# ska-sa/dc_sand

Hardware: AMD Instinct MI355X
Metric: Gcoeff/s (complex weights) 64ant x 1024beam x 32768chan per GPU (higher is better)
Workload: dtype f32

## Files before the change

### dc_sand_amd/csrc/bf_capi.hip

```cpp

#include "../../include/dcs_beamformer.h"
#ifdef DCS_PROBES
#include "../../include/dcs_probes.h"
#endif

#include <hip/hip_runtime.h>

#include <cmath>
#include <cstdio>
#include <cstdlib>
#include <cstring>
#include <new>

#include "../../include/dcs_stream_staging.h"
#include "bf_kernels.h"
#include "bf_ctx_ext.h"
#include "bf_stream_ext.h"

static_assert(sizeof(dcs_delay_vals) == 16, "delay_vals must be 4 x fp32 (BeamformerParameters.h:61-66)");

#define DCS_TRY(expr)                          \
    do {                                       \
        hipError_t _e = (expr);                \
        if (_e != hipSuccess) return (int)_e;  \
// ... 43 lines not shown
    k.dHalfChannels = p->nr_channels / 2.0;
    k.dDenominator = (double)D;
    return k;
}

int verify_div3(dcs_bf_consts *k)
{
    uint32_t *d_cnt = nullptr;
    uint32_t h_cnt = 1;
    hipError_t e = hipMalloc((void **)&d_cnt, sizeof(uint32_t));
    if (e != hipSuccess) return (int)e;
    e = hipMemset(d_cnt, 0, sizeof(uint32_t));
    if (e == hipSuccess) e = bf_launch_verify_div3(k->fDenominator, k->fRcpDenominator, d_cnt, nullptr);
    if (e == hipSuccess) e = hipMemcpy(&h_cnt, d_cnt, sizeof(uint32_t), hipMemcpyDeviceToHost);
    (void)hipFree(d_cnt);
    if (e != hipSuccess) return (int)e;
    k->uDiv3Exact = (h_cnt == 0u) ? 1u : 0u;
    return DCS_OK;
}

}

constexpr int kSideStreams = 4;
struct dcs_bf_context {
    bf_ctx_ext_head ext;
    dcs_bf_params p;
    dcs_bf_consts k;
    uint32_t n_pairs;
    int device;
    uint32_t div3_verified;
    bool tuning_now;
    dcs_delay_vals *d_table[2];
    int cur;
    bool table_set;
    float *d_dt;
    float *h_dt;
    hipEvent_t dt_ev[kDtSlots];
    hipStream_t side[kSideStreams];
    hipEvent_t fork_ev, join_ev[kSideStreams];
    bool dt_used[kDtSlots];
    int dt_next;
    uint32_t pairs_pad;
    uint32_t terms_steps;
    float *d_terms;
    uint32_t *d_flags;
    uint32_t flag_epoch;
    float *d_wnorm;
    float *d_wscale;
    float *d_tt_terms;
    uint32_t *d_tt_flags;
    dcs_bf_tuning tune;
    struct tuned_geom {
        bool valid;
        int32_t tpb, cpb, wpc;
    } tuned[3][2];
#ifdef DCS_PROBES
    dcs_probe_knobs probe;
#endif
};
#ifdef DCS_PROBES
#define DCS_PROBE_KNOB(c, f) ((c)->probe.f)
#else
#define DCS_PROBE_KNOB(c, f) 0
#endif

constexpr int kTableRing = 4;
struct dcs_bf_stream {
    bf_stream_ext_head ext;
    dcs_bf_context *ctx;
    hipStream_t stream;
    hipGraph_t graph;
    hipGraphExec_t exec;
    hipGraphNode_t node;
    bf_kernel_launch launch;
    bool has_terms;
    hipGraphNode_t terms_node;
    bf_terms_args terms_args;
    const void *terms_func;
    dim3 terms_grid, terms_block;
    dcs_delay_vals *h_table[kTableRing];
    hipEvent_t table_copied[kTableRing];
    bool table_pending[kTableRing];
    int table_next;
    hipGraph_t ggraph;
    hipGraphExec_t gexec;
    hipGraphNode_t gnode_gather, gnode_terms, gnode_gen;
    bf_gather_launch gather;
    dcs_delay_vals *d_spare;
    hipStream_t stage_stream;
    hipEvent_t staged_ev;
    hipEvent_t released_ev;
    bool released_recorded;
    bool staged;
};

extern "C" {

const char *dcs_error_string(int status)
{
    switch (status) {
    case DCS_OK: return "dcs: success";
    case DCS_ERR_INVALID_ARGUMENT: return "dcs error: invalid argument";
    case DCS_ERR_UNSUPPORTED: return "dcs error: this kernel does not support the requested mode";
    case DCS_ERR_NOT_READY: return "dcs error: not ready (no delay table set)";
    case DCS_ERR_OUT_OF_RANGE: return "dcs error: out of range";
    case DCS_ERR_NO_DEVICE: return "dcs error: no HIP device";
    case DCS_ERR_WRONG_DEVICE: return "dcs error: the context belongs to another device than the current one (dcs_device_set)";
    default: break;
    }
    if (status > 0) return hipGetErrorString((hipError_t)status);
    return "dcs error: unknown status";
}

int dcs_abi_version(void) { return DCS_BF_ABI_VERSION; }

int dcs_bf_default_params(dcs_bf_params *p)
{
    if (!p) return DCS_ERR_INVALID_ARGUMENT;
    p->nr_channels = 64;
    p->nr_stations = 64;
    p->nr_beams = 16;
    p->nr_samples_per_channel = 256;
    p->sampling_period = 1e-7f;
    p->fft_size = 8192;
    p->adc_sample_rate = 1712e6;
    p->accumulations_before_new_coeffs = 256;
    p->reserved = 0;
    return DCS_OK;
}

int dcs_bf_output_bytes(const dcs_bf_params *p, int bitwidth, uint32_t nt, size_t *bytes)
{
    if (!params_ok(p) || !bytes) return DCS_ERR_INVALID_ARGUMENT;
    if (bitwidth != DCS_BF_B16 && bitwidth != DCS_BF_B32) return DCS_ERR_INVALID_ARGUMENT;
    const size_t elem = bitwidth == DCS_BF_B16 ? sizeof(uint16_t) : sizeof(float);
    *bytes = (size_t)nt * (size_t)p->nr_channels * (size_t)p->nr_stations * (size_t)p->nr_beams * 2u * elem;
    return DCS_OK;
}

int dcs_bf_delta_times(const dcs_bf_params *p, uint64_t t0, uint32_t nt, float *dt_out)
{
    if (!params_ok(p) || (!dt_out && nt)) return DCS_ERR_INVALID_ARGUMENT;
    for (uint32_t i = 0; i < nt; i++) {
        const uint64_t t = t0 + i;
        volatile float a = (float)t;
        volatile float b = a * p->sampling_period;
        volatile float c = b * 1e9f;
        volatile float d = c * (float)p->fft_size;
        if (!(d < 9.2e18f)) return DCS_ERR_OUT_OF_RANGE;
        const long step_ns = (long)d;
        volatile float num = (float)step_ns;
        volatile float q = num / 1e9f;
        volatile float dt = 0.0f + q;
        dt_out[i] = dt;
    }
    return DCS_OK;
}

int dcs_bf_ts_diff(const struct timespec *first, const struct timespec *last, float *dt_out)
{
    if (!first || !last || !dt_out) return DCS_ERR_INVALID_ARGUMENT;
    volatile float fl = (float)last->tv_sec, ff = (float)first->tv_sec;
    volatile float secs = fl - ff;
    const long nanosec_difference = last->tv_nsec - first->tv_nsec;
    volatile float num = (float)nanosec_difference;
    volatile float q = num / 1e9f;
    volatile float dt = secs + q;
    *dt_out = dt;
    return DCS_OK;
}
// ... 1045 lines not shown
            float ms = 0.0f;
            if (st == 0) st = time_launches(n_timed, &ms);
            if (st == 0 && ms / n_timed < cands[i].best_ms) cands[i].best_ms = ms / n_timed;
        }
    }
    int order[40];
    for (int i = 0; i < ncand; i++) order[i] = i;
    for (int i = 0; i < ncand; i++)
        for (int j = i + 1; j < ncand; j++)
            if (cands[order[j]].best_ms < cands[order[i]].best_ms) { const int t = order[i]; order[i] = order[j]; order[j] = t; }
    int finalists[5];
    int nfinal = 0;
    for (int i = 0; i < ncand && nfinal < 4; i++)
        if (order[i] != i_default) finalists[nfinal++] = order[i];
    finalists[nfinal++] = i_default;
    double final_ms[5] = {0.0, 0.0, 0.0, 0.0, 0.0};
    const int n_final = (int)std::fmin(800.0, std::fmax(8.0, std::ceil(12.0 / one)));
    for (int rnd = 0; rnd < 3 && st == 0; rnd++) {
        for (int f = 0; f < nfinal && st == 0; f++) {
            use(cands[finalists[f]]);
            for (int i = 0; i < n_settle && st == 0; i++) st = dcs_bf_generate_slab(c, bitwidth, 1, nt_tune, 0, nc, d_out, out_bytes, stream);
            float ms = 0.0f;
            if (st == 0) st = time_launches(n_final, &ms);
            final_ms[f] += ms / n_final;
        }
    }
    if (e0) (void)hipEventDestroy(e0);
    if (e1) (void)hipEventDestroy(e1);
    int best = i_default;
    double best_ms = final_ms[nfinal - 1] / 1.007;
    for (int f = 0; f + 1 < nfinal && st == 0; f++)
        if (final_ms[f] < best_ms) { best_ms = final_ms[f]; best = finalists[f]; }
    if (st == 0) {
        use(cands[best]);
        for (int k = 0; k < n_settle && st == 0; k++) st = dcs_bf_generate_slab(c, bitwidth, 1, nt_tune, 0, nc, d_out, out_bytes, stream);
    }
    c->tune = saved;
    c->tuning_now = false;
    if (st != 0) return st;
    slot.valid = true;
    slot.tpb = cands[best].tpb;
    slot.cpb = cands[best].cpb;
    slot.wpc = cands[best].wpc;
    report();
    return DCS_OK;
}

int dcs_bf_gpu_utilisation(const dcs_bf_params *p, float kernel_ms, float out[2])
{
    if (!params_ok(p) || !out) return DCS_ERR_INVALID_ARGUMENT;
    const float fRateOfFFTs_Hz = ((float)p->adc_sample_rate) / ((float)p->fft_size);
    const float fTransferTimePerPacket_s = 1 / fRateOfFFTs_Hz;
    float single = (kernel_ms / 1000.0) / (p->nr_samples_per_channel * fTransferTimePerPacket_s);
    float multiple = single / ((float)p->accumulations_before_new_coeffs);
    single *= 4;
    multiple *= 4;
    out[0] = single;
    out[1] = multiple;
    return DCS_OK;
}

namespace {

void kernel_node_params(const bf_kernel_launch &l, void **params, hipKernelNodeParams *np)
{
    std::memset(np, 0, sizeof(*np));
    np->func = const_cast<void *>(l.func);
    np->gridDim = l.grid;
    np->blockDim = l.block;
    np->sharedMemBytes = l.shared;
    np->kernelParams = params;
    np->extra = nullptr;
}

void terms_node_params(const dcs_bf_stream *s, void **params, hipKernelNodeParams *tp)
{
    std::memset(tp, 0, sizeof(*tp));
    tp->func = const_cast<void *>(s->terms_func);
    tp->gridDim = s->terms_grid;
    tp->blockDim = s->terms_block;
    tp->kernelParams = params;
}

void gather_node_params(dcs_bf_stream *s, void **params, hipKernelNodeParams *gp)
{
    bf_gather_launch &g = s->gather;
    params[0] = &g.local;
    params[1] = &g.global;
    params[2] = &g.n_ant;
    params[3] = &g.nb_local;
    params[4] = &g.nb_total;
    params[5] = &g.beam_offset;
    std::memset(gp, 0, sizeof(*gp));
    gp->func = const_cast<void *>(g.func);
    gp->gridDim = g.grid;
    gp->blockDim = g.block;
    gp->kernelParams = params;
}

int build_stream_graph(dcs_bf_stream *s, bool with_gather, hipGraph_t *graph, hipGraphExec_t *exec, hipGraphNode_t *n_gather,
                       hipGraphNode_t *n_terms, hipGraphNode_t *n_gen)
{
    DCS_TRY(hipGraphCreate(graph, 0));
    hipGraphNode_t prev = nullptr;
    if (with_gather) {
        void *gparams[6];
        hipKernelNodeParams gp;
        gather_node_params(s, gparams, &gp);
        DCS_TRY(hipGraphAddKernelNode(n_gather, *graph, nullptr, 0, &gp));
        prev = *n_gather;
    }
    if (s->has_terms) {
        void *tparams[] = {&s->terms_args};
        hipKernelNodeParams tp;
        terms_node_params(s, tparams, &tp);
        DCS_TRY(hipGraphAddKernelNode(n_terms, *graph, prev ? &prev : nullptr, prev ? 1 : 0, &tp));
        prev = *n_terms;
    }
    void *params[] = {&s->launch.args};
    hipKernelNodeParams np;
    kernel_node_params(s->launch, params, &np);
    DCS_TRY(hipGraphAddKernelNode(n_gen, *graph, prev ? &prev : nullptr, prev ? 1 : 0, &np));
    DCS_TRY(hipGraphInstantiate(exec, *graph, nullptr, nullptr, 0));
    return DCS_OK;
}

int replay(dcs_bf_stream *s, float dt, const dcs_delay_vals *delays, hipGraphExec_t exec, hipGraphNode_t n_gather,
           hipGraphNode_t n_terms, hipGraphNode_t n_gen)
{
    s->launch.args.a.dt0 = dt;
    s->launch.args.a.delays = delays;
    if (n_gather) {
        void *gparams[6];
        hipKernelNodeParams gp;
        gather_node_params(s, gparams, &gp);
        DCS_TRY(hipGraphExecKernelNodeSetParams(exec, n_gather, &gp));
    }
    if (s->has_terms) {
        s->terms_args.dt0 = dt;
        s->terms_args.dt_inline[0] = dt;
        s->terms_args.delays = delays;
        void *tparams[] = {&s->terms_args};
        hipKernelNodeParams tp;
        terms_node_params(s, tparams, &tp);
        DCS_TRY(hipGraphExecKernelNodeSetParams(exec, n_terms, &tp));
    }
    void *params[] = {&s->launch.args};
    hipKernelNodeParams np;
    kernel_node_params(s->launch, params, &np);
    DCS_TRY(hipGraphExecKernelNodeSetParams(exec, n_gen, &np));
    return (int)hipGraphLaunch(exec, s->stream);
}

int ensure_staging(dcs_bf_stream *s)
{
    if (!s->d_spare) DCS_TRY(hipMalloc((void **)&s->d_spare, (size_t)s->ctx->n_pairs * sizeof(dcs_delay_vals)));
    if (!s->stage_stream) {
        int least = 0, greatest = 0;
        DCS_TRY(hipDeviceGetStreamPriorityRange(&least, &greatest));
        DCS_TRY(hipStreamCreateWithPriority(&s->stage_stream, hipStreamNonBlocking, greatest));
    }
    if (!s->staged_ev) DCS_TRY(hipEventCreateWithFlags(&s->staged_ev, hipEventDisableTiming));
    if (!s->released_ev) DCS_TRY(hipEventCreateWithFlags(&s->released_ev, hipEventDisableTiming));
    return DCS_OK;
}

int begin_staging(dcs_bf_stream *s)
{
    const int cap = refuse_if_capturing(s->stream);
    if (cap != DCS_OK) return cap;
    const int st = ensure_staging(s);
    if (st != DCS_OK) return st;
    if (s->released_recorded) DCS_TRY(hipStreamWaitEvent(s->stage_stream, s->released_ev, 0));
    return DCS_OK;
}

int consume_staged(dcs_bf_stream *s, float dt)
{
    dcs_bf_context *c = s->ctx;
    DCS_TRY(hipStreamWaitEvent(s->stream, s->staged_ev, 0));
    DCS_TRY(hipEventRecord(s->released_ev, s->stream));
    s->released_recorded = true;
    const int st = replay(s, dt, s->d_spare, s->exec, nullptr, s->terms_node, s->node);
    if (st != DCS_OK) return st;
    dcs_delay_vals *retired = c->d_table[c->cur];
    c->d_table[c->cur] = s->d_spare;
    s->d_spare = retired;
    s->staged = false;
    return DCS_OK;
}

int stage_table_impl(dcs_bf_stream *s, const dcs_delay_vals *table, int flags)
{
    if (!s || !table) return DCS_ERR_INVALID_ARGUMENT;
    if (flags != 0 && flags != DCS_BF_STAGE_CALLER_PINNED) return DCS_ERR_INVALID_ARGUMENT;
    dcs_bf_context *c = s->ctx;
    DCS_CHECK_DEVICE(c);
    const size_t tb = (size_t)c->n_pairs * sizeof(dcs_delay_vals);
    const int st = begin_staging(s);
    if (st != DCS_OK) return st;
    const void *src = table;
    int r = -1;
    if (flags == 0) {
        r = s->table_next;
        s->table_next = (r + 1) % kTableRing;
        if (s->table_pending[r]) DCS_TRY(hipEventSynchronize(s->table_copied[r]));
        std::memcpy(s->h_table[r], table, tb);
        src = s->h_table[r];
    }
    DCS_TRY(hipMemcpyAsync(s->d_spare, src, tb, hipMemcpyHostToDevice, s->stage_stream));
    if (r >= 0) {
        DCS_TRY(hipEventRecord(s->table_copied[r], s->stage_stream));
        s->table_pending[r] = true;
    }
    DCS_TRY(hipEventRecord(s->staged_ev, s->stage_stream));
    s->staged = true;
    return DCS_OK;
}

int stage_table_from_global_impl(dcs_bf_stream *s, const void *d_global, uint32_t nb_total, uint32_t beam_offset,
                                 void *ready_event)
{
    if (!s || !d_global) return DCS_ERR_INVALID_ARGUMENT;
    dcs_bf_context *c = s->ctx;
    DCS_CHECK_DEVICE(c);
    if ((uint64_t)beam_offset + (uint64_t)c->p.nr_beams > nb_total) return DCS_ERR_OUT_OF_RANGE;
    if ((reinterpret_cast<uintptr_t>(d_global) & 15u) != 0) return DCS_ERR_INVALID_ARGUMENT;
    const int st = begin_staging(s);
    if (st != DCS_OK) return st;
    if (ready_event) DCS_TRY(hipStreamWaitEvent(s->stage_stream, reinterpret_cast<hipEvent_t>(ready_event), 0));
    DCS_TRY(bf_launch_gather_beams(s->d_spare, static_cast<const dcs_delay_vals *>(d_global), (uint32_t)c->p.nr_stations,
                                   (uint32_t)c->p.nr_beams, nb_total, beam_offset, s->stage_stream));
    DCS_TRY(hipEventRecord(s->staged_ev, s->stage_stream));
    s->staged = true;
    return DCS_OK;
}

const bf_stream_ext_ops kStagingOps = {BF_STREAM_EXT_VERSION, stage_table_impl, stage_table_from_global_impl};

}

int dcs_bf_stream_begin(dcs_bf_context *c, int bitwidth, uint32_t c0, uint32_t nc, void *d_out, size_t out_bytes,
                        void *stream, dcs_bf_stream **out)
{
    if (!c || !out || !d_out) return DCS_ERR_INVALID_ARGUMENT;
    DCS_CHECK_DEVICE(c);
    *out = nullptr;
    if (bitwidth != DCS_BF_B16 && bitwidth != DCS_BF_B32) return DCS_ERR_INVALID_ARGUMENT;
    if (!c->table_set) return DCS_ERR_NOT_READY;
    if ((uint64_t)c0 + nc > (uint64_t)c->p.nr_channels || nc == 0) return DCS_ERR_OUT_OF_RANGE;
    const bool out16 = bitwidth == DCS_BF_B16;
    if (out_bytes < (size_t)nc * c->n_pairs * (out16 ? 4 : 8)) return DCS_ERR_INVALID_ARGUMENT;
    {
        const int cap = refuse_if_capturing(as_stream(stream));
        if (cap != DCS_OK) return cap;
    }

    dcs_bf_stream *s = new (std::nothrow) dcs_bf_stream();
    if (!s) return (int)hipErrorOutOfMemory;
    std::memset(static_cast<void *>(s), 0, sizeof(*s));
    s->ext.ops = &kStagingOps;
    s->ctx = c;
    s->stream = as_stream(stream);
    int st = DCS_OK;
    do {
        s->has_terms = want_terms_table(c, out16, pick_geometry(c, out16, nc, 1), nc, 1);
        if ((st = prepare_tiled(c, out16, nullptr, 0.0f, 1, c0, nc, d_out, &s->launch, nullptr, s->has_terms)) != 0) break;
        if (s->launch.func == nullptr) { st = DCS_ERR_INVALID_ARGUMENT; break; }
        if (s->has_terms) {
            fill_terms_table_args(c, out16, 0.0f, 1, c0, nc, d_out, nullptr, &s->terms_args);
            if ((st = (int)bf_prepare_terms(s->terms_args, &s->terms_func, &s->terms_grid, &s->terms_block)) != 0) break;
            if (s->terms_func == nullptr) { st = DCS_ERR_INVALID_ARGUMENT; break; }
        }
        if ((st = (int)bf_prepare_gather_beams(c->d_table[c->cur ^ 1], c->d_table[c->cur], (uint32_t)c->p.nr_stations,
                                               (uint32_t)c->p.nr_beams, (uint32_t)c->p.nr_beams, 0u, &s->gather)) != 0) break;
        if (s->gather.func == nullptr) { st = DCS_ERR_INVALID_ARGUMENT; break; }
        for (int i = 0; i < kTableRing && st == 0; i++) {
            st = (int)hipHostMalloc((void **)&s->h_table[i], (size_t)c->n_pairs * sizeof(dcs_delay_vals), hipHostMallocDefault);
            if (st == 0) st = (int)hipEventCreateWithFlags(&s->table_copied[i], hipEventDisableTiming);
        }
        if (st != 0) break;
        if ((st = build_stream_graph(s, false, &s->graph, &s->exec, nullptr, &s->terms_node, &s->node)) != 0) break;
        if ((st = build_stream_graph(s, true, &s->ggraph, &s->gexec, &s->gnode_gather, &s->gnode_terms, &s->gnode_gen)) != 0) break;
    } while (0);
    if (st != 0) {
        dcs_bf_stream_end(s);
        return st;
    }
    *out = s;
    return DCS_OK;
}

int dcs_bf_stream_tick_dt(dcs_bf_stream *s, float dt, const dcs_delay_vals *new_table)
{
    if (!s) return DCS_ERR_INVALID_ARGUMENT;
    dcs_bf_context *c = s->ctx;
    DCS_CHECK_DEVICE(c);
    if (s->staged) return new_table ? DCS_ERR_INVALID_ARGUMENT : consume_staged(s, dt);
    if (new_table) {
        const int r = s->table_next;
        s->table_next = (r + 1) % kTableRing;
        if (s->table_pending[r]) DCS_TRY(hipEventSynchronize(s->table_copied[r]));
        std::memcpy(s->h_table[r], new_table, (size_t)c->n_pairs * sizeof(dcs_delay_vals));
        const int nxt = c->cur ^ 1;
        DCS_TRY(hipMemcpyAsync(c->d_table[nxt], s->h_table[r], (size_t)c->n_pairs * sizeof(dcs_delay_vals),
                               hipMemcpyHostToDevice, s->stream));
        DCS_TRY(hipEventRecord(s->table_copied[r], s->stream));
        s->table_pending[r] = true;
        c->cur = nxt;
    }
    return replay(s, dt, c->d_table[c->cur], s->exec, nullptr, s->terms_node, s->node);
}

int dcs_bf_stream_tick(dcs_bf_stream *s, uint64_t t, const dcs_delay_vals *new_table)
{
    if (!s) return DCS_ERR_INVALID_ARGUMENT;
    float dt;
    const int st = dcs_bf_delta_times(&s->ctx->p, t, 1, &dt);
    if (st != DCS_OK) return st;
    return dcs_bf_stream_tick_dt(s, dt, new_table);
}

int dcs_bf_stream_tick_at(dcs_bf_stream *s, const struct timespec *cur, const struct timespec *ref,
                          const dcs_delay_vals *new_table)
{
    if (!s) return DCS_ERR_INVALID_ARGUMENT;
    float dt;
    const int st = dcs_bf_ts_diff(ref, cur, &dt);
    if (st != DCS_OK) return st;
    return dcs_bf_stream_tick_dt(s, dt, new_table);
}

int dcs_bf_stream_tick_dt_from_global(dcs_bf_stream *s, float dt, const void *d_global, uint32_t nb_total, uint32_t beam_offset)
{
    if (!s || !d_global) return DCS_ERR_INVALID_ARGUMENT;
    dcs_bf_context *c = s->ctx;
    DCS_CHECK_DEVICE(c);
    if ((uint64_t)beam_offset + (uint64_t)c->p.nr_beams > nb_total) return DCS_ERR_OUT_OF_RANGE;
    if ((reinterpret_cast<uintptr_t>(d_global) & 15u) != 0) return DCS_ERR_INVALID_ARGUMENT;
    if (s->staged) return DCS_ERR_INVALID_ARGUMENT;
    const int nxt = c->cur ^ 1;
    s->gather.local = c->d_table[nxt];
    s->gather.global = static_cast<const dcs_delay_vals *>(d_global);
    s->gather.nb_total = nb_total;
    s->gather.beam_offset = beam_offset;
    c->cur = nxt;
    return replay(s, dt, c->d_table[c->cur], s->gexec, s->gnode_gather, s->gnode_terms, s->gnode_gen);
}

int dcs_bf_stream_tick_from_global(dcs_bf_stream *s, uint64_t t, const void *d_global, uint32_t nb_total, uint32_t beam_offset)
{
    if (!s) return DCS_ERR_INVALID_ARGUMENT;
    float dt;
    const int st = dcs_bf_delta_times(&s->ctx->p, t, 1, &dt);
    if (st != DCS_OK) return st;
    return dcs_bf_stream_tick_dt_from_global(s, dt, d_global, nb_total, beam_offset);
}

int dcs_bf_stream_tick_at_from_global(dcs_bf_stream *s, const struct timespec *cur, const struct timespec *ref,
                                      const void *d_global, uint32_t nb_total, uint32_t beam_offset)
{
    if (!s) return DCS_ERR_INVALID_ARGUMENT;
    float dt;
    const int st = dcs_bf_ts_diff(ref, cur, &dt);
    if (st != DCS_OK) return st;
    return dcs_bf_stream_tick_dt_from_global(s, dt, d_global, nb_total, beam_offset);
}

int dcs_bf_stream_end(dcs_bf_stream *s)
{
    if (!s) return DCS_OK;
    (void)hipStreamSynchronize(s->stream);
    if (s->stage_stream) {
        (void)hipStreamSynchronize(s->stage_stream);
        (void)hipStreamDestroy(s->stage_stream);
    }
    if (s->staged_ev) (void)hipEventDestroy(s->staged_ev);
    if (s->released_ev) (void)hipEventDestroy(s->released_ev);
    if (s->d_spare) (void)hipFree(s->d_spare);
    if (s->exec) (void)hipGraphExecDestroy(s->exec);
    if (s->graph) (void)hipGraphDestroy(s->graph);
    if (s->gexec) (void)hipGraphExecDestroy(s->gexec);
    if (s->ggraph) (void)hipGraphDestroy(s->ggraph);
    for (int i = 0; i < kTableRing; i++) {
        if (s->table_copied[i]) (void)hipEventDestroy(s->table_copied[i]);
        if (s->h_table[i]) (void)hipHostFree(s->h_table[i]);
    }
    delete s;
    return DCS_OK;
}

#ifdef DCS_PROBES
int dcs_probe_set_knobs(dcs_bf_context *c, const dcs_probe_knobs *k)
{
    if (!c) return DCS_ERR_INVALID_ARGUMENT;
    if (!k) {
        std::memset(&c->probe, 0, sizeof(c->probe));
        return DCS_OK;
    }
    if (k->pace < 0 || k->pace > 4096 || k->fail_at_step < 0) return DCS_ERR_INVALID_ARGUMENT;
    c->probe = *k;
    return DCS_OK;
}
#endif

}
```

### dc_sand_amd/csrc/bf_kernels.h

```cpp
#ifndef DCS_BF_KERNELS_H
#define DCS_BF_KERNELS_H

#include <hip/hip_runtime.h>
#include <stdint.h>

#include "bf_math.h"

struct bf_tiled_args {
    const dcs_delay_vals *delays;
    void *out;
    const float *dt_dev;
    float dt0;
    uint32_t n_pairs;
    uint32_t c0, nc;
    uint32_t nt;
    uint32_t chan_per_block;
    uint32_t n_tile_groups;
    uint32_t n_cblocks;
    uint32_t xcd_remap;
#ifdef DCS_PROBES
    uint32_t pace;
#endif
    dcs_bf_consts k;
    const float *terms;
    const uint32_t *flags;
    uint32_t pairs_pad;
};
constexpr uint32_t kDtInline = 256;
struct bf_tiled_args_inl {
    bf_tiled_args a;
    float dt_inline[kDtInline];
};

struct bf_kernel_launch {
    const void *func;
    dim3 grid, block;
    uint32_t shared;
    bf_tiled_args_inl args;
};
hipError_t bf_prepare_tiled(const bf_tiled_args &a, const float *dt_inline, bool out16, int tiles_per_block,
                            bool nontemporal, bf_kernel_launch *out);

struct bf_terms_args {
    const dcs_delay_vals *delays;
    float *terms;
    uint32_t *flags;
    const float *dt_dev;
    float dt0;
    uint32_t n_pairs, pairs_pad, nt;
    dcs_bf_consts k;
    float dt_inline[8];
    void *out;
    uint32_t c0, nc, out16;
};
constexpr uint32_t kTermsInline = 8;
hipError_t bf_launch_terms(const bf_terms_args &a, hipStream_t stream);
hipError_t bf_prepare_terms(const bf_terms_args &a, const void **func, dim3 *grid, dim3 *block);

struct bf_rows_args {
    const float *terms;
    const uint32_t *flags;
    void *out;
    uint32_t n_pairs, pairs_pad;
    uint32_t c0, nc, nt;
    uint32_t n_colgroups, n_rowgroups;
    uint32_t xcd_remap;
    uint32_t div3;
    uint32_t same_tile;
#ifdef DCS_PROBES
    uint32_t pace;
#endif
    uint32_t lds_pad;
    float D, y;
};
hipError_t bf_launch_rows(const bf_rows_args &a, bool out16, int waves_per_block, int rows_per_wave,
                          bool nontemporal, bool xcd_remap, bool nomath, hipStream_t stream);

struct bf_bform_terms_args {
    const dcs_delay_vals *delays;
    float *terms;
    uint32_t *flags;
    uint32_t epoch;
    const float *dt_dev;
    float dt0;
    uint32_t n_pairs, A, B, nt;
    dcs_bf_consts k;
};
struct bf_bform_terms_args_inl {
    bf_bform_terms_args a;
    float dt_inline[kDtInline];
};
hipError_t bf_launch_bform_terms(const bf_bform_terms_args &a, const float *dt_inline, hipStream_t stream);

struct bf_weights_args {
    const float *g;
    float *gn;
    float *gs;
};
hipError_t bf_launch_bform_terms_weighted(const bf_bform_terms_args &a, const bf_weights_args &w, const float *dt_inline,
                                          hipStream_t stream);

struct bf_beamform_args {
    const float *terms;
    const uint32_t *flags;
    uint32_t epoch;
    const int8_t *ant;
    float *beams;
    uint32_t A, B, C;
    uint32_t nt16;
    uint32_t tex0;
    uint32_t nt16_total;
    uint32_t chan_per_block;
    uint32_t n_bgroups, n_cblocks;
    dcs_bf_consts k;
};
hipError_t bf_launch_beamform(const bf_beamform_args &a, hipStream_t stream);
hipError_t bf_launch_beamform_weighted(const bf_beamform_args &a, const bf_weights_args &w, hipStream_t stream);

struct bf_bacc_args {
    const float *terms;
    const uint32_t *flags;
    uint32_t epoch;
    const int8_t *ant;
    float *beams;
    uint32_t A, B, C, nT16;
    uint32_t fp32_chain;
    uint32_t share_off;
#ifdef DCS_PROBES
    uint32_t max_rounds;
    uint32_t no_share;
    uint32_t plain_stores;
    uint32_t wg_per_cu;
    uint32_t unstaged;
    uint32_t order;
    uint32_t nbt_force;
    uint32_t nw_force;
// ... 51 lines not shown
```

### dc_sand_amd/csrc/bf_kernels.hip

```cpp

#include "bf_kernels.h"

#include <hip/hip_runtime.h>

#include <cstring>
#include <type_traits>

#include "bf_device.h"

namespace {

template <bool OUT16, int TPB, bool NT, bool ALIGNED, bool NOMATH, int TAG = 0, bool INL = false, bool TERMS = false, bool HALF = false>
__global__ void __launch_bounds__(kBlock) bf_tiled_kernel(const std::conditional_t<INL, bf_tiled_args_inl, bf_tiled_args> args)
{
    const bf_tiled_args &a = [&]() -> const bf_tiled_args & {
        if constexpr (INL)
            return args.a;
        else
            return args;
    }();
    constexpr int PPL = OUT16 ? 4 : 2;
    constexpr int TILE = 64 * PPL;
    constexpr int ROWS = 4 / TPB;
    constexpr uint32_t EB = OUT16 ? 4u : 8u;
    constexpr int kSlowUnroll = OUT16 ? 1 : PPL;

    uint32_t bid = blockIdx.x;
    if (a.xcd_remap) bid = (bid % 8u) * (gridDim.x / 8u) + bid / 8u;
    const uint32_t tg = bid % a.n_tile_groups;
    const uint32_t rest = bid / a.n_tile_groups;
    const uint32_t cb = rest % a.n_cblocks;
    const uint32_t t = rest / a.n_cblocks;
    const uint32_t pair_base = tg * (uint32_t)(TPB * TILE);

    const uint32_t wave = HALF ? (uint32_t)__builtin_amdgcn_readfirstlane(threadIdx.x >> 6) : threadIdx.x >> 6;
    const uint32_t lane = threadIdx.x & 63u;
    const uint32_t tile = wave % TPB;
    const uint32_t row = wave / TPB;
    const uint32_t li = tile * TILE + lane * PPL;
    const uint32_t p0 = pair_base + li;

    float fRate[PPL], fPhase0[PPL];
    bool wave_slow, wave_low;
    if constexpr (TERMS) {
        const uint32_t wave_p0 = pair_base + tile * (uint32_t)TILE;
        uint32_t cls = DCS_CLASS_FAST_LOW;
        if (wave_p0 < a.pairs_pad) {
            const uint32_t *fl = a.flags + (uint64_t)t * (a.pairs_pad / 64u) + wave_p0 / 64u;
#pragma unroll
            for (int j = 0; j < TILE / 64; j++)
                if (wave_p0 + 64u * (uint32_t)j < a.pairs_pad) cls = max(cls, fl[j]);
        }
        cls = __builtin_amdgcn_readfirstlane(cls);
        wave_slow = false;
        wave_low = cls == DCS_CLASS_FAST_LOW;
        if (cls == DCS_CLASS_SLOW) return;
        if (p0 >= a.n_pairs) return;
        const floatx4 *tp = reinterpret_cast<const floatx4 *>(a.terms + 2u * ((uint64_t)t * a.pairs_pad + p0));
#pragma unroll
        for (int j = 0; j < PPL; j += 2) {
            const floatx4 v = tp[j / 2];
            fRate[j] = v.x;
            fPhase0[j] = v.y;
            fRate[j + 1] = v.z;
            fPhase0[j + 1] = v.w;
        }
    } else {
        __shared__ __attribute__((aligned(16))) float s_terms[TPB * TILE * 2];
        float dt;
        if constexpr (INL)
            dt = a.dt_dev ? a.dt_dev[t] : args.dt_inline[t];
        else
            dt = a.dt_dev ? a.dt_dev[t] : a.dt0;

        for (uint32_t i = threadIdx.x; i < (uint32_t)(TPB * TILE); i += kBlock) {
            const uint32_t p = pair_base + i;
            float fR = 0.0f, fP = 0.0f;
            if (p < a.n_pairs) {
                const floatx4 raw = *reinterpret_cast<const floatx4 *>(&a.delays[p]);
                dcs_delay_vals d;
                d.fDelay_s = raw.x;
                d.fDelayRate_sps = raw.y;
                d.fPhase_rad = raw.z;
                d.fPhaseRate_radps = raw.w;
                dcs_pair_terms(d, dt, a.k.dHalfChannels, a.k.dDenominator, &fR, &fP);
            }
            *reinterpret_cast<floatx2 *>(&s_terms[2 * i]) = floatx2{fR, fP};
        }
        __syncthreads();

        uint32_t cls = DCS_CLASS_FAST_LOW;
#pragma unroll
        for (int j = 0; j < PPL; j += 2) {
            const floatx4 v = *reinterpret_cast<const floatx4 *>(&s_terms[2 * (li + j)]);
            fRate[j] = v.x;
            fPhase0[j] = v.y;
            fRate[j + 1] = v.z;
            fPhase0[j + 1] = v.w;
        }
#pragma unroll
        for (int j = 0; j < PPL; j++) cls = max(cls, dcs_pair_class(fRate[j], fPhase0[j], a.k.fRotBoundScale, a.k.fLowDegLimit));
        wave_slow = __builtin_amdgcn_ballot_w64(cls == DCS_CLASS_SLOW) != 0ull;
        wave_low = __builtin_amdgcn_ballot_w64(cls != DCS_CLASS_FAST_LOW) == 0ull;
    }

    const uint32_t cbeg = cb * a.chan_per_block;
    const uint32_t cend = min(cbeg + a.chan_per_block, a.nc);
    if (p0 >= a.n_pairs) return;

    const float D = a.k.fDenominator, y = a.k.fRcpDenominator;
    const uint64_t row_bytes = (uint64_t)a.n_pairs * EB;
    char *dst = reinterpret_cast<char *>(a.out) +
                ((uint64_t)t * a.nc + (cbeg + row)) * row_bytes + (uint64_t)p0 * EB;
    const uint64_t step = (uint64_t)ROWS * row_bytes;

    auto emit = [&](const float (&re)[PPL], const float (&im)[PPL]) {
        if constexpr (ALIGNED) {
            if constexpr (OUT16) {
                uintx4 v;
                v.x = pack_half2(re[0], im[0]);
                v.y = pack_half2(re[1], im[1]);
                v.z = pack_half2(re[2], im[2]);
                v.w = pack_half2(re[3], im[3]);
                store_global<NT>(reinterpret_cast<uintx4 *>(dst), v);
            } else {
                store_global<NT>(reinterpret_cast<floatx4 *>(dst), floatx4{re[0], im[0], re[1], im[1]});
            }
        } else {
#pragma unroll
            for (int j = 0; j < PPL; j++) {
                if (p0 + j < a.n_pairs) {
                    if constexpr (OUT16)
                        store_global<NT>(reinterpret_cast<uint32_t *>(dst) + j, pack_half2(re[j], im[j]));
                    else
                        store_global<NT>(reinterpret_cast<floatx2 *>(dst) + j, floatx2{re[j], im[j]});
                }
            }
        }
    };

    if constexpr (NOMATH) {
        float re[PPL], im[PPL];
#pragma unroll
        for (int j = 0; j < PPL; j++) {
            re[j] = fRate[j];
            im[j] = fPhase0[j];
        }
        for (uint32_t c = cbeg + row; c < cend; c += ROWS) {
            emit(re, im);
            dst += step;
        }
        return;
    }

    static_assert(!HALF || OUT16, "the binary16-sized arithmetic is for b16 output");
    if (HALF && !wave_slow) {
        if constexpr (HALF) {
            auto walk = [&](auto div3) {
                for (uint32_t c = cbeg + row; c < cend; c += ROWS) {
                    const float fChan = (float)(a.c0 + c);
                    uint32_t w[PPL];
#pragma unroll
// ... 91 lines not shown
    for (int j = 0; j < PPL; j += 2) {
        const floatx4 v = tp[j / 2];
        fRate[j] = v.x;
        fPhase0[j] = v.y;
        fRate[j + 1] = v.z;
        fPhase0[j + 1] = v.w;
    }
    if (p0 >= a.n_pairs) return;

    const float D = a.D, y = a.y;
    const uint64_t row_bytes = (uint64_t)a.n_pairs * EB;
    char *dst = reinterpret_cast<char *>(a.out) + ((uint64_t)t * a.nc + c) * row_bytes + (uint64_t)p0 * EB;

    auto emit = [&](const float (&re)[PPL], const float (&im)[PPL]) {
        if constexpr (ALIGNED) {
            if constexpr (OUT16) {
                uintx4 v;
                v.x = pack_half2(re[0], im[0]);
                v.y = pack_half2(re[1], im[1]);
                v.z = pack_half2(re[2], im[2]);
                v.w = pack_half2(re[3], im[3]);
                store_global<NT>(reinterpret_cast<uintx4 *>(dst), v);
            } else {
                store_global<NT>(reinterpret_cast<floatx4 *>(dst), floatx4{re[0], im[0], re[1], im[1]});
            }
        } else {
#pragma unroll
            for (int j = 0; j < PPL; j++) {
                if (p0 + j < a.n_pairs) {
                    if constexpr (OUT16)
                        store_global<NT>(reinterpret_cast<uint32_t *>(dst) + j, pack_half2(re[j], im[j]));
                    else
                        store_global<NT>(reinterpret_cast<floatx2 *>(dst) + j, floatx2{re[j], im[j]});
                }
            }
        }
    };

    if (__builtin_expect(cls != DCS_CLASS_SLOW, 1)) {
        dispatch_fast(a.div3 != 0u, cls == DCS_CLASS_FAST_LOW, [&](auto div3, auto lowdeg) {
#pragma unroll
            for (int r = 0; r < RPW; r++) {
                if (c + r * row_step < a.nc) {
                    const float fChan = (float)(a.c0 + c + r * row_step);
                    float re[PPL], im[PPL];
#pragma unroll
                    for (int j = 0; j < PPL; j++) {
                        if constexpr (NOMATH) {
                            re[j] = fRate[j];
                            im[j] = fPhase0[j] + fChan;
                        } else {
                            coeff_fast<decltype(div3)::value, decltype(lowdeg)::value>(fRate[j], fPhase0[j], fChan, D, y, re[j], im[j]);
                        }
                    }
#ifdef DCS_PROBES
                    for (uint32_t k = 0; k < a.pace; k++) __builtin_amdgcn_s_sleep(1);
#endif
                    emit(re, im);
                    dst += row_bytes * row_step;
                }
            }
        });
    } else {
        for (int r = 0; r < RPW; r++) {
            if (c + r * row_step < a.nc) {
                const float fChan = (float)(a.c0 + c + r * row_step);
                float re[PPL], im[PPL];
#pragma unroll 1
                for (int j = 0; j < PPL; j++) coeff_slow(fRate[j], fPhase0[j], fChan, D, re[j], im[j]);
                emit(re, im);
                dst += row_bytes * row_step;
            }
        }
    }
}

__global__ void __launch_bounds__(kBlock) bf_terms_kernel(const bf_terms_args a)
{
    const uint32_t p = blockIdx.x * kBlock + threadIdx.x;
    const uint32_t t = blockIdx.y;
    const float dt = a.dt_dev ? a.dt_dev[t] : a.dt_inline[t];
    float fRate = 0.0f, fPhase0 = 0.0f;
    if (p < a.n_pairs) {
        const floatx4 raw = *reinterpret_cast<const floatx4 *>(&a.delays[p]);
        dcs_delay_vals d;
        d.fDelay_s = raw.x;
        d.fDelayRate_sps = raw.y;
        d.fPhase_rad = raw.z;
        d.fPhaseRate_radps = raw.w;
        dcs_pair_terms(d, dt, a.k.dHalfChannels, a.k.dDenominator, &fRate, &fPhase0);
    }
    const uint32_t cls = dcs_pair_class(fRate, fPhase0, a.k.fRotBoundScale, a.k.fLowDegLimit);
    uint32_t wave_cls = __builtin_amdgcn_ballot_w64(cls == DCS_CLASS_SLOW) != 0ull
                            ? DCS_CLASS_SLOW
                            : (__builtin_amdgcn_ballot_w64(cls == DCS_CLASS_FAST_HIGH) != 0ull ? DCS_CLASS_FAST_HIGH
                                                                                              : DCS_CLASS_FAST_LOW);
    if (a.out != nullptr) {
        if (__syncthreads_or((int)(cls == DCS_CLASS_SLOW))) {
            wave_cls = DCS_CLASS_SLOW;
            if (p < a.n_pairs) {
                const uint64_t eb = a.out16 ? 4u : 8u;
                char *dst = reinterpret_cast<char *>(a.out) + ((uint64_t)t * a.nc * a.n_pairs + p) * eb;
                for (uint32_t c = 0; c < a.nc; c++) {
                    float re, im;
                    coeff_slow(fRate, fPhase0, (float)(a.c0 + c), a.k.fDenominator, re, im);
                    if (a.out16)
                        *reinterpret_cast<uint32_t *>(dst) = pack_half2(re, im);
                    else
                        *reinterpret_cast<floatx2 *>(dst) = floatx2{re, im};
                    dst += (uint64_t)a.n_pairs * eb;
                }
            }
        }
    }
    *reinterpret_cast<floatx2 *>(a.terms + 2u * ((uint64_t)t * a.pairs_pad + p)) = floatx2{fRate, fPhase0};
    if ((threadIdx.x & 63u) == 0u) a.flags[(uint64_t)t * (a.pairs_pad / 64u) + p / 64u] = wave_cls;
}

template <bool INL>
using bf_bform_terms_param = std::conditional_t<INL, bf_bform_terms_args_inl, bf_bform_terms_args>;
template <bool INL>
struct bf_bform_terms_wargs {
    bf_bform_terms_param<INL> t;
    bf_weights_args w;
};

__device__ __forceinline__ void bform_weights_row(const bf_bform_terms_args &a, const bf_weights_args &w)
{
    const uint32_t lane = threadIdx.x & 63u;
    const uint32_t waves = gridDim.x * (kBlock / 64u);
    for (uint32_t beam = blockIdx.x * (kBlock / 64u) + (threadIdx.x >> 6); beam < a.B; beam += waves) {
        const float *g = w.g + (uint64_t)beam * a.A;
        float m = 0.0f;
        bool bad = false;
        float v[4];
#pragma unroll
        for (uint32_t k = 0; k < 4; k++) {
            const uint32_t ant = lane + 64u * k;
            v[k] = ant < a.A ? g[ant] : 0.0f;
        }
        auto note = [&](float x) {
            x = fabsf(x);
            m = fmaxf(m, x);
            bad |= !(x <= 3.40282347e38f);
        };
#pragma unroll
        for (uint32_t k = 0; k < 4; k++) note(v[k]);
        for (uint32_t ant = lane + 256u; ant < a.A; ant += 64u) note(g[ant]);
#pragma unroll
        for (int off = 32; off > 0; off >>= 1) m = fmaxf(m, __shfl_xor(m, off));
        const float s = __builtin_amdgcn_ballot_w64(bad) != 0u ? __builtin_nanf("") : m;
        auto ghat = [&](float x) { return s == 0.0f ? 0.0f : __fdiv_rn(x, s); };
#pragma unroll
        for (uint32_t k = 0; k < 4; k++) {
            const uint32_t ant = lane + 64u * k;
            if (ant < a.A) w.gn[(uint64_t)ant * a.B + beam] = ghat(v[k]);
        }
        for (uint32_t ant = lane + 256u; ant < a.A; ant += 64u) w.gn[(uint64_t)ant * a.B + beam] = ghat(g[ant]);
        if (lane == 0u) w.gs[beam] = s;
    }
}

template <bool INL, bool WEIGHTED>
__device__ __forceinline__ void bform_terms_body(const bf_bform_terms_param<INL> &args, const bf_weights_args &w)
{
    const bf_bform_terms_args &a = [&]() -> const bf_bform_terms_args & {
        if constexpr (INL)
// ... 426 lines not shown
```

Before: 916.9.

## Fuse global delay-table gather into terms/generator kernels and drop gather graph

Removes the separate gather kernel node and second graph. The terms or tiled kernel now reads delays directly from the global multi-beam table through a source descriptor, and one designated block or slice writes the local copy. The new-table path on the host now reuses the staging stream and event handoff instead of an inline ring memcpy, and the staging events are created without a system fence. The aim is to cut a kernel launch and a graph dependency per tick, at the cost of extra index arithmetic and a branch inside the kernels' load path.

```diff
diff --git a/dc_sand_amd/csrc/bf_capi.hip b/dc_sand_amd/csrc/bf_capi.hip
--- a/dc_sand_amd/csrc/bf_capi.hip
+++ b/dc_sand_amd/csrc/bf_capi.hip
@@ -149,10 +149,6 @@
     hipEvent_t table_copied[kTableRing];
     bool table_pending[kTableRing];
     int table_next;
-    hipGraph_t ggraph;
-    hipGraphExec_t gexec;
-    hipGraphNode_t gnode_gather, gnode_terms, gnode_gen;
-    bf_gather_launch gather;
     dcs_delay_vals *d_spare;
     hipStream_t stage_stream;
     hipEvent_t staged_ev;
@@ -1364,34 +1360,10 @@
     tp->kernelParams = params;
 }
 
-void gather_node_params(dcs_bf_stream *s, void **params, hipKernelNodeParams *gp)
-{
-    bf_gather_launch &g = s->gather;
-    params[0] = &g.local;
-    params[1] = &g.global;
-    params[2] = &g.n_ant;
-    params[3] = &g.nb_local;
-    params[4] = &g.nb_total;
-    params[5] = &g.beam_offset;
-    std::memset(gp, 0, sizeof(*gp));
-    gp->func = const_cast<void *>(g.func);
-    gp->gridDim = g.grid;
-    gp->blockDim = g.block;
-    gp->kernelParams = params;
-}
-
-int build_stream_graph(dcs_bf_stream *s, bool with_gather, hipGraph_t *graph, hipGraphExec_t *exec, hipGraphNode_t *n_gather,
-                       hipGraphNode_t *n_terms, hipGraphNode_t *n_gen)
+int build_stream_graph(dcs_bf_stream *s, hipGraph_t *graph, hipGraphExec_t *exec, hipGraphNode_t *n_terms, hipGraphNode_t *n_gen)
 {
     DCS_TRY(hipGraphCreate(graph, 0));
     hipGraphNode_t prev = nullptr;
-    if (with_gather) {
-        void *gparams[6];
-        hipKernelNodeParams gp;
-        gather_node_params(s, gparams, &gp);
-        DCS_TRY(hipGraphAddKernelNode(n_gather, *graph, nullptr, 0, &gp));
-        prev = *n_gather;
-    }
     if (s->has_terms) {
         void *tparams[] = {&s->terms_args};
         hipKernelNodeParams tp;
@@ -1407,31 +1379,32 @@
     return DCS_OK;
 }
 
-int replay(dcs_bf_stream *s, float dt, const dcs_delay_vals *delays, hipGraphExec_t exec, hipGraphNode_t n_gather,
-           hipGraphNode_t n_terms, hipGraphNode_t n_gen)
-{
+int replay(dcs_bf_stream *s, float dt, const dcs_delay_vals *delays, const bf_table_src *src = nullptr)
+{
+    const bf_table_src none{};
     s->launch.args.a.dt0 = dt;
     s->launch.args.a.delays = delays;
-    if (n_gather) {
-        void *gparams[6];
-        hipKernelNodeParams gp;
-        gather_node_params(s, gparams, &gp);
-        DCS_TRY(hipGraphExecKernelNodeSetParams(exec, n_gather, &gp));
-    }
     if (s->has_terms) {
         s->terms_args.dt0 = dt;
         s->terms_args.dt_inline[0] = dt;
         s->terms_args.delays = delays;
+        s->terms_args.src = src ? *src : none;
         void *tparams[] = {&s->terms_args};
         hipKernelNodeParams tp;
         terms_node_params(s, tparams, &tp);
-        DCS_TRY(hipGraphExecKernelNodeSetParams(exec, n_terms, &tp));
+        const hipError_t e = hipGraphExecKernelNodeSetParams(s->exec, s->terms_node, &tp);
+        s->terms_args.src = none;
+        DCS_TRY(e);
+    } else {
+        s->launch.args.a.src = src ? *src : none;
     }
     void *params[] = {&s->launch.args};
     hipKernelNodeParams np;
     kernel_node_params(s->launch, params, &np);
-    DCS_TRY(hipGraphExecKernelNodeSetParams(exec, n_gen, &np));
-    return (int)hipGraphLaunch(exec, s->stream);
+    const hipError_t e = hipGraphExecKernelNodeSetParams(s->exec, s->node, &np);
+    s->launch.args.a.src = none;
+    DCS_TRY(e);
+    return (int)hipGraphLaunch(s->exec, s->stream);
 }
 
 int ensure_staging(dcs_bf_stream *s)
@@ -1442,8 +1415,9 @@
         DCS_TRY(hipDeviceGetStreamPriorityRange(&least, &greatest));
         DCS_TRY(hipStreamCreateWithPriority(&s->stage_stream, hipStreamNonBlocking, greatest));
     }
-    if (!s->staged_ev) DCS_TRY(hipEventCreateWithFlags(&s->staged_ev, hipEventDisableTiming));
-    if (!s->released_ev) DCS_TRY(hipEventCreateWithFlags(&s->released_ev, hipEventDisableTiming));
+    const unsigned ev_flags = hipEventDisableTiming | hipEventDisableSystemFence;
+    if (!s->staged_ev) DCS_TRY(hipEventCreateWithFlags(&s->staged_ev, ev_flags));
+    if (!s->released_ev) DCS_TRY(hipEventCreateWithFlags(&s->released_ev, ev_flags));
     return DCS_OK;
 }
 
@@ -1463,7 +1437,7 @@
     DCS_TRY(hipStreamWaitEvent(s->stream, s->staged_ev, 0));
     DCS_TRY(hipEventRecord(s->released_ev, s->stream));
     s->released_recorded = true;
-    const int st = replay(s, dt, s->d_spare, s->exec, nullptr, s->terms_node, s->node);
+    const int st = replay(s, dt, s->d_spare);
     if (st != DCS_OK) return st;
     dcs_delay_vals *retired = c->d_table[c->cur];
     c->d_table[c->cur] = s->d_spare;
@@ -1554,16 +1528,12 @@
             if ((st = (int)bf_prepare_terms(s->terms_args, &s->terms_func, &s->terms_grid, &s->terms_block)) != 0) break;
             if (s->terms_func == nullptr) { st = DCS_ERR_INVALID_ARGUMENT; break; }
         }
-        if ((st = (int)bf_prepare_gather_beams(c->d_table[c->cur ^ 1], c->d_table[c->cur], (uint32_t)c->p.nr_stations,
-                                               (uint32_t)c->p.nr_beams, (uint32_t)c->p.nr_beams, 0u, &s->gather)) != 0) break;
-        if (s->gather.func == nullptr) { st = DCS_ERR_INVALID_ARGUMENT; break; }
         for (int i = 0; i < kTableRing && st == 0; i++) {
             st = (int)hipHostMalloc((void **)&s->h_table[i], (size_t)c->n_pairs * sizeof(dcs_delay_vals), hipHostMallocDefault);
             if (st == 0) st = (int)hipEventCreateWithFlags(&s->table_copied[i], hipEventDisableTiming);
         }
         if (st != 0) break;
-        if ((st = build_stream_graph(s, false, &s->graph, &s->exec, nullptr, &s->terms_node, &s->node)) != 0) break;
-        if ((st = build_stream_graph(s, true, &s->ggraph, &s->gexec, &s->gnode_gather, &s->gnode_terms, &s->gnode_gen)) != 0) break;
+        if ((st = build_stream_graph(s, &s->graph, &s->exec, &s->terms_node, &s->node)) != 0) break;
     } while (0);
     if (st != 0) {
         dcs_bf_stream_end(s);
@@ -1579,19 +1549,12 @@
     dcs_bf_context *c = s->ctx;
     DCS_CHECK_DEVICE(c);
     if (s->staged) return new_table ? DCS_ERR_INVALID_ARGUMENT : consume_staged(s, dt);
-    if (new_table) {
-        const int r = s->table_next;
-        s->table_next = (r + 1) % kTableRing;
-        if (s->table_pending[r]) DCS_TRY(hipEventSynchronize(s->table_copied[r]));
-        std::memcpy(s->h_table[r], new_table, (size_t)c->n_pairs * sizeof(dcs_delay_vals));
-        const int nxt = c->cur ^ 1;
-        DCS_TRY(hipMemcpyAsync(c->d_table[nxt], s->h_table[r], (size_t)c->n_pairs * sizeof(dcs_delay_vals),
-                               hipMemcpyHostToDevice, s->stream));
-        DCS_TRY(hipEventRecord(s->table_copied[r], s->stream));
-        s->table_pending[r] = true;
-        c->cur = nxt;
-    }
-    return replay(s, dt, c->d_table[c->cur], s->exec, nullptr, s->terms_node, s->node);
+    if (!new_table) return replay(s, dt, c->d_table[c->cur]);
+    int st = stage_table_impl(s, new_table, 0);
+    if (st != DCS_OK) return st;
+    st = consume_staged(s, dt);
+    if (st != DCS_OK) s->staged = false;
+    return st;
 }
 
 int dcs_bf_stream_tick(dcs_bf_stream *s, uint64_t t, const dcs_delay_vals *new_table)
@@ -1622,12 +1585,16 @@
     if ((reinterpret_cast<uintptr_t>(d_global) & 15u) != 0) return DCS_ERR_INVALID_ARGUMENT;
     if (s->staged) return DCS_ERR_INVALID_ARGUMENT;
     const int nxt = c->cur ^ 1;
-    s->gather.local = c->d_table[nxt];
-    s->gather.global = static_cast<const dcs_delay_vals *>(d_global);
-    s->gather.nb_total = nb_total;
-    s->gather.beam_offset = beam_offset;
+    bf_table_src src{};
+    src.global = static_cast<const dcs_delay_vals *>(d_global);
+    src.copy = c->d_table[nxt];
+    src.nb_local = (uint32_t)c->p.nr_beams;
+    src.nb_total = nb_total;
+    src.beam_offset = beam_offset;
+    const int st = replay(s, dt, c->d_table[nxt], &src);
+    if (st != DCS_OK) return st;
     c->cur = nxt;
-    return replay(s, dt, c->d_table[c->cur], s->gexec, s->gnode_gather, s->gnode_terms, s->gnode_gen);
+    return DCS_OK;
 }
 
 int dcs_bf_stream_tick_from_global(dcs_bf_stream *s, uint64_t t, const void *d_global, uint32_t nb_total, uint32_t beam_offset)
@@ -1662,8 +1629,6 @@
     if (s->d_spare) (void)hipFree(s->d_spare);
     if (s->exec) (void)hipGraphExecDestroy(s->exec);
     if (s->graph) (void)hipGraphDestroy(s->graph);
-    if (s->gexec) (void)hipGraphExecDestroy(s->gexec);
-    if (s->ggraph) (void)hipGraphDestroy(s->ggraph);
     for (int i = 0; i < kTableRing; i++) {
         if (s->table_copied[i]) (void)hipEventDestroy(s->table_copied[i]);
         if (s->h_table[i]) (void)hipHostFree(s->h_table[i]);
diff --git a/dc_sand_amd/csrc/bf_kernels.h b/dc_sand_amd/csrc/bf_kernels.h
--- a/dc_sand_amd/csrc/bf_kernels.h
+++ b/dc_sand_amd/csrc/bf_kernels.h
@@ -5,6 +5,12 @@
 #include <stdint.h>
 
 #include "bf_math.h"
+
+struct bf_table_src {
+    const dcs_delay_vals *global;
+    dcs_delay_vals *copy;
+    uint32_t nb_local, nb_total, beam_offset;
+};
 
 struct bf_tiled_args {
     const dcs_delay_vals *delays;
@@ -25,6 +31,7 @@
     const float *terms;
     const uint32_t *flags;
     uint32_t pairs_pad;
+    bf_table_src src;
 };
 constexpr uint32_t kDtInline = 256;
 struct bf_tiled_args_inl {
@@ -52,6 +59,7 @@
     float dt_inline[8];
     void *out;
     uint32_t c0, nc, out16;
+    bf_table_src src;
 };
 constexpr uint32_t kTermsInline = 8;
 hipError_t bf_launch_terms(const bf_terms_args &a, hipStream_t stream);
diff --git a/dc_sand_amd/csrc/bf_kernels.hip b/dc_sand_amd/csrc/bf_kernels.hip
--- a/dc_sand_amd/csrc/bf_kernels.hip
+++ b/dc_sand_amd/csrc/bf_kernels.hip
@@ -9,6 +9,15 @@
 #include "bf_device.h"
 
 namespace {
+
+__device__ __forceinline__ floatx4 load_delays(const dcs_delay_vals *delays, const bf_table_src &src, uint32_t p, bool copy)
+{
+    if (src.global == nullptr) return *reinterpret_cast<const floatx4 *>(&delays[p]);
+    const uint32_t ant = p / src.nb_local, b = p - ant * src.nb_local;
+    const floatx4 v = *reinterpret_cast<const floatx4 *>(&src.global[(uint64_t)ant * src.nb_total + src.beam_offset + b]);
+    if (copy) *reinterpret_cast<floatx4 *>(&src.copy[p]) = v;
+    return v;
+}
 
 template <bool OUT16, int TPB, bool NT, bool ALIGNED, bool NOMATH, int TAG = 0, bool INL = false, bool TERMS = false, bool HALF = false>
 __global__ void __launch_bounds__(kBlock) bf_tiled_kernel(const std::conditional_t<INL, bf_tiled_args_inl, bf_tiled_args> args)
@@ -77,7 +86,7 @@
             const uint32_t p = pair_base + i;
             float fR = 0.0f, fP = 0.0f;
             if (p < a.n_pairs) {
-                const floatx4 raw = *reinterpret_cast<const floatx4 *>(&a.delays[p]);
+                const floatx4 raw = load_delays(a.delays, a.src, p, cb == 0u && t == 0u);
                 dcs_delay_vals d;
                 d.fDelay_s = raw.x;
                 d.fDelayRate_sps = raw.y;
@@ -335,7 +344,7 @@
     const float dt = a.dt_dev ? a.dt_dev[t] : a.dt_inline[t];
     float fRate = 0.0f, fPhase0 = 0.0f;
     if (p < a.n_pairs) {
-        const floatx4 raw = *reinterpret_cast<const floatx4 *>(&a.delays[p]);
+        const floatx4 raw = load_delays(a.delays, a.src, p, t == 0u);
         dcs_delay_vals d;
         d.fDelay_s = raw.x;
         d.fDelayRate_sps = raw.y;
```

Result: no change. 917.2 (median of 5 runs) (+0.0%).
